# lucianpls/QB3

Measured on AMD Instinct MI355X. Metric: MPixel/s encode+decode (QB3M_FTL, 8-bit 3-band), higher is better.
Workload: dtype u8; 1 GPU; 16384x16384x3 uint8 NOISY3 seed 2; QB3M_FTL qb3x_encode_device (self-indexed container, table level 2) + qb3x_decode_device of that container alone (index = NULL, restart table inside the container); table_level=2, container_bytes=458870207

## Files before the change

### include/qb3x.h

```cpp
#ifndef QB3_AMD_QB3X_H
#define QB3_AMD_QB3X_H
#include "QB3.h"

#if defined(__cplusplus)
extern "C" {
#endif

int qb3x_device_count(void);

void qb3x_trim(void);

unsigned qb3x_last_decode_status(const decsp p);

size_t qb3x_index_size(const encsp p);
size_t qb3x_decoder_index_size(const decsp p);

size_t qb3x_encode_device(encsp p, const void *d_src, void *d_dst, void *d_index, void *stream);

size_t qb3x_decode_device(decsp p, const void *d_src, void *d_dst, const void *d_index, void *stream);

size_t qb3x_decode_window_device(decsp p, const void *d_src, const void *d_index, size_t x0, size_t y0, size_t w, size_t h,
                                 void *d_dst, size_t dst_stride, void *stream);
size_t qb3x_read_window(decsp p, size_t x0, size_t y0, size_t w, size_t h, void *dst, size_t dst_stride);
size_t qb3x_window_segments(const decsp p, size_t x0, size_t y0, size_t w, size_t h, size_t *blocks_per_segment);
int    qb3x_last_window_path(const decsp p);
size_t qb3x_last_window_segments(const decsp p);
#define QB3X_WINK_U16 1u
#define QB3X_WINK_CF8 2u
#define QB3X_WINK_UNIT 4u
#define QB3X_WINK_CFU 8u
void qb3x_set_decoder_window_kernels(decsp p, unsigned mask);

// ... 75 lines not shown
```

### qb3_amd/__init__.py

```python
import ctypes as C
import os

_HERE = os.path.dirname(os.path.abspath(__file__))
LIB_PATH = os.environ.get("QB3_LIB_PATH") or os.path.join(_HERE, "libQB3.so")

if not os.path.exists(LIB_PATH):
    raise ImportError(f"{LIB_PATH} not built: run `python -c 'import __graft_entry__ as g; g.build()'` "
                      "or `make -C qb3_amd/csrc` (there is no CPU fallback)")

try:
    import torch as _torch
except ImportError:
    _torch = None

lib = C.CDLL(LIB_PATH)

QB3_U8, QB3_I8, QB3_U16, QB3_I16, QB3_U32, QB3_I32, QB3_U64, QB3_I64 = range(8)
QB3M_BASE_Z, QB3M_CF, QB3M_RLE, QB3M_CF_RLE, QB3M_BASE_H, QB3M_CF_H, QB3M_RLE_H, QB3M_CF_RLE_H, QB3M_FTL = range(9)
QB3M_DEFAULT, QB3M_BASE, QB3M_BEST, QB3M_STORED, QB3M_INVALID = 8, 4, 7, 255, -1
QB3X_REF_CBAND0 = 1
QB3X_WINK_U16 = 1
QB3X_WINK_CF8 = 2
QB3X_WINK_UNIT = 4
QB3X_WINK_CFU = 8
# ... 35 lines not shown
    "qb3_read_info": (C.c_bool, [_vp]),
    "qb3_read_data": (_sz, [_vp, _vp]),
    "qb3_destroy_decoder": (None, [_vp]),
    "qb3_decoded_size": (_sz, [_vp]),
    "qb3_get_type": (C.c_int, [_vp]),
    "qb3_set_decoder_stride": (None, [_vp, _sz]),
    "qb3_get_mode": (C.c_int, [_vp]),
    "qb3_get_quanta": (_u64, [_vp]),
    "qb3_get_order": (_u64, [_vp]),
    "qb3_get_coreband": (C.c_bool, [_vp, C.POINTER(_sz)]),
    "qb3x_device_count": (C.c_int, []),
    "qb3x_trim": (None, []),
    "qb3x_last_decode_status": (C.c_uint, [_vp]),
    "qb3x_index_size": (_sz, [_vp]),
    "qb3x_set_encoder_index_chunk": (None, [_vp, C.c_int]),
    "qb3x_decoder_index_size": (_sz, [_vp]),
    "qb3x_encode_device": (_sz, [_vp, _vp, _vp, _vp, _vp]),
    "qb3x_decode_device": (_sz, [_vp, _vp, _vp, _vp, _vp]),
    "qb3x_encode_tiles": (_sz, [_vp, _vp, _sz, _sz, _vp, _sz, _vp, C.POINTER(_sz), _vp]),
    "qb3x_decode_tiles": (_sz, [_vp, _vp, _sz, _sz, C.POINTER(_sz), _vp, _sz, _vp, _vp]),
    "qb3x_decode_tile_ok": (C.c_int, [_vp, _sz]),
    "qb3x_mosaic_tiles": (_sz, [_sz, _sz, _sz, _sz, C.POINTER(_sz), C.POINTER(_sz)]),
    "qb3x_encode_mosaic": (_sz, [_vp, _vp, _sz, _sz, _sz, _vp, _sz, _vp, C.POINTER(_sz), _vp]),
    "qb3x_decode_mosaic": (_sz, [_vp, _vp, _sz, C.POINTER(_sz), _sz, _sz, _vp, _sz, _vp, _vp]),
    "qb3x_mosaic_window_tiles": (_sz, [_sz] * 8 + [C.POINTER(_sz)] * 4),
    "qb3x_decode_mosaic_windows": (_sz, [_vp, _vp, _sz, C.POINTER(_sz), _sz, _sz, _vp, _sz, _vp]),
    "qb3x_last_mosaic_whole_tiles": (_sz, [_vp]),
    "qb3x_decode_window_device": (_sz, [_vp, _vp, _vp, _sz, _sz, _sz, _sz, _vp, _sz, _vp]),
    "qb3x_read_window": (_sz, [_vp, _sz, _sz, _sz, _sz, _vp, _sz]),
    "qb3x_window_segments": (_sz, [_vp, _sz, _sz, _sz, _sz, C.POINTER(_sz)]),
# ... 266 lines not shown
```

### qb3_amd/csrc/api_mem.cpp

```cpp
#include <chrono>
#include <mutex>
#include "qb3_host.h"

using namespace qb3dev;
using namespace qb3api;

struct DevPool {
    struct Item { void *p; size_t cap; int dev; };
    static constexpr size_t POOL_ITEMS = 24;
    const size_t POOL_BYTES = [] { const char *e = getenv("QB3_POOL_MB"); return (e && e[0] ? (size_t)strtoull(e, nullptr, 10) : (size_t)3072) << 20; }();
    std::mutex mu;
    std::vector<Item> items;
    size_t bytes = 0;
    void *take(size_t n, int dev, size_t *cap) {
        std::lock_guard<std::mutex> l(mu);
        size_t best = items.size();
        for (size_t i = 0; i < items.size(); i++)
            if (items[i].dev == dev && items[i].cap >= n && items[i].cap / 2 <= n && (best == items.size() || items[i].cap < items[best].cap)) best = i;
        if (best == items.size()) return nullptr;
        void *p = items[best].p;
        *cap = items[best].cap;
        bytes -= items[best].cap;
        items.erase(items.begin() + (long)best);
        return p;
// ... 50 lines not shown
}
QB3_API void qb3x_trim(void) { try { dev_pool().trim(); qb3host::ring_trim(); } catch (...) {} }

bool qb3api::device_ok() {
    int n = 0;
    hipError_t e = hipGetDeviceCount(&n);
    if (e != hipSuccess || n <= 0) { set_error("no usable HIP device (the block codec has no CPU fallback)", (int)e); return false; }
    return true;
}

hipError_t qb3api::wait_stream(hipStream_t st) {
    const auto t0 = std::chrono::steady_clock::now();
    for (uint32_t i = 0;; i++) {
        const hipError_t e = hipStreamQuery(st);
        if (e != hipErrorNotReady) return e;
        if ((i & 63) == 63 && std::chrono::steady_clock::now() - t0 > std::chrono::milliseconds(4)) break;
    }
    return hipStreamSynchronize(st);
}
hipError_t qb3api::fetch_small(void *dst, const void *d_src, size_t n, hipStream_t st) {
    static thread_local void *pinned = nullptr;
    if (!pinned && hipHostMalloc(&pinned, 1024, hipHostMallocDefault) != hipSuccess) pinned = nullptr;
    if (!pinned || n > 1024) {
        hipError_t e = hipMemcpyAsync(dst, d_src, n, hipMemcpyDeviceToHost, st);
        return e == hipSuccess ? hipStreamSynchronize(st) : e;
    }
    hipError_t e = hipMemcpyAsync(pinned, d_src, n, hipMemcpyDeviceToHost, st);
    if (e == hipSuccess) e = wait_stream(st);
    if (e == hipSuccess) memcpy(dst, pinned, n);
    return e;
}

static void parallel_memcpy(uint8_t *dst, const uint8_t *src, size_t n) {
// ... 73 lines not shown
```

### qb3_amd/csrc/api_tiles.cpp

```cpp
#include "qb3_host.h"

using namespace qb3dev;
using namespace qb3api;

static const uint8_t *grid_img(const TileGrid &G, size_t u) { return (const uint8_t *)G.img + (u / G.cols) * G.img_row + (u % G.cols) * G.img_col; }
static size_t grid_k(const TileGrid &G, size_t u) { return G.k0 + (u / G.cols) * G.k_row + u % G.cols; }
static size_t grid_piece(const TileGrid &G, size_t first, size_t batch, uint32_t *cols) {
    const size_t c = first % G.cols;
    if (c == 0 && batch >= G.cols) {
        *cols = (uint32_t)G.cols;
        return std::min(batch / G.cols, (G.n - first) / G.cols) * G.cols;
    }
    *cols = 0;
    return std::min(batch, G.cols - c);
}
template <class H> struct StrideGuard {
    H *p; size_t saved;
    explicit StrideGuard(H *h) : p(h), saved(h->stride) {}
    ~StrideGuard() { p->stride = saved; }
};

static size_t encode_tiles_loop(encsp p, const TileGrid &G, size_t first, size_t n, void *d_dst, size_t dst_pitch,
                                void *d_index, size_t isz, size_t *sizes, void *stream, qb3_mode mode) {
    size_t done = 0;
// ... 2 lines not shown
        qb3_reset_encoder(p);
        p->mode = mode;
        sizes[k] = qb3x_encode_device(p, grid_img(G, u), (uint8_t *)d_dst + k * dst_pitch,
                                      d_index ? (uint8_t *)d_index + k * isz : nullptr, stream);
        done += sizes[k] != 0;
    }
    return done;
}

size_t qb3api::encode_tile_grids(encsp p, const TileGrid *grids, size_t ngrids, void *d_dst, size_t dst_pitch,
                                 void *d_index, size_t *sizes, void *stream) {
    const size_t isz = d_index ? qb3x_index_size(p) : 0;
    const qb3_mode mode = p->mode;
    const size_t tsz = szof(p->type);
    hipStream_t st = (hipStream_t)stream;
    StrideGuard<encs> keep(p);
    size_t nmax = 0;
    for (size_t gi = 0; gi < ngrids; gi++) nmax = std::max(nmax, grids[gi].n);
    const bool batchable = !is_rle_mode(mode) && mode != QB3M_STORED && p->quanta < 2 && p->xsize >= 4 && p->ysize >= 4 &&
                           p->xsize * p->ysize > 16 && !p->error && device_ok();
    if (!batchable) {
        size_t k = 0;
        for (size_t gi = 0; gi < ngrids; gi++) {
            p->stride = grids[gi].stride;
            k += encode_tiles_loop(p, grids[gi], 0, grids[gi].n, d_dst, dst_pitch, d_index, isz, sizes, stream, mode);
        }
        if (mode != QB3M_STORED) p->mode = mode;
        return k;
    }

// ... 205 lines not shown
```

### qb3_amd/csrc/k_enc_post.hip

```cpp
#include "qb3_kernels.h"
#include "qb3_ix_fill.h"

namespace qb3dev {

__global__ void __launch_bounds__(SCAN_GROUP / 4) enc_scan_kernel(const EncArgs a0) {
    const EncArgs a = enc_for_tile(a0, blockIdx.y);
    __shared__ uint32_t wsum[16];
    __shared__ uint64_t wsum64[16];
    __shared__ uint64_t carry;
    __shared__ uint32_t is_last;
    const uint32_t tid = threadIdx.x, i0 = blockIdx.x * SCAN_GROUP + 4 * tid;
    const uint32_t ngroups = (a.nchunks + SCAN_GROUP - 1) / SCAN_GROUP;
    uint32_t v[4], sum = 0;
#pragma unroll
    for (int k = 0; k < 4; k++) { v[k] = (i0 + k < a.nchunks) ? a.chunk_bits[i0 + k] : 0; sum += v[k]; }
    uint32_t total;
    uint64_t off = block_exscan(sum, wsum, &total);
#pragma unroll
    for (int k = 0; k < 4; k++) if (i0 + k < a.nchunks) { a.chunk_off[i0 + k] = off; off += v[k]; }
    if (tid == 0) {
        a.group_sum[blockIdx.x] = total;
        __threadfence();
        is_last = atomicAdd((uint32_t *)&a.group_sum[ngroups + 1], 1u) == gridDim.x - 1;
        carry = 0;
    }
    __syncthreads();
    if (!is_last) return;
    __threadfence();
    for (uint32_t base = 0; base < ngroups; base += blockDim.x) {
        const uint32_t i = base + tid;
        const uint64_t g = i < ngroups ? __hip_atomic_load(&a.group_sum[i], __ATOMIC_RELAXED, __HIP_MEMORY_SCOPE_AGENT) : 0ull;
        const uint64_t ex = block_exscan_v<uint64_t>(g, wsum64);
        const uint64_t c0 = carry;
        if (i < ngroups) a.group_sum[i] = c0 + ex;
        __syncthreads();
        if (tid == blockDim.x - 1) carry = c0 + ex + g;
        __syncthreads();
    }
    if (tid == 0) { a.group_sum[ngroups] = carry; a.res->zero_run = 0; a.res->ff_pairs = 0; a.res->zero_dwords = 0; }
}

__device__ __forceinline__ uint64_t chunk_start(const EncArgs &a, uint32_t k) {
    if (k >= a.nchunks) return a.group_sum[(a.nchunks + SCAN_GROUP - 1) / SCAN_GROUP];
    return a.group_sum[k / SCAN_GROUP] + a.chunk_off[k];
}

__device__ __forceinline__ uint32_t zero_runs_in(uint32_t cur, uint32_t nxt) {
    return (uint32_t)(cur == 0) + (uint32_t)(__builtin_amdgcn_alignbit(nxt, cur, 8) == 0) +
           (uint32_t)(__builtin_amdgcn_alignbit(nxt, cur, 16) == 0) + (uint32_t)(__builtin_amdgcn_alignbit(nxt, cur, 24) == 0);
}
__device__ __forceinline__ uint32_t ff_pairs_in(uint32_t v) {
    const uint32_t t = v & (v >> 8) & 0x00ffffffu;
    return (uint32_t)__popc(((t & 0x7f7f7fu) + 0x010101u) & t & 0x808080u);
}
// ... 326 lines not shown
```

### qb3_amd/csrc/k_host.hip

```cpp
#include "qb3_kernels.h"
#include "qb3_walk.h"

namespace qb3dev {

static thread_local char g_err[256] = "";
const char *last_error() { return g_err; }
void set_error(const char *what, int e) {
    snprintf(g_err, sizeof(g_err), "%s: %s", what, e ? hipGetErrorString((hipError_t)e) : "failed");
}

const Tuning &tuning() {
    static const Tuning t = [] {
        auto on = [](const char *name) { const char *e = getenv(name); return e && e[0] && e[0] != '0'; };
        Tuning v;
        v.no_px = on("QB3_NO_PX");
        v.slow_walk = on("QB3_SLOW_WALK");
        const char *cap = getenv("QB3_WALK_TAB_KB");
        v.walk_tab_kb = cap ? (size_t)strtoull(cap, nullptr, 10) : 0;
        v.slow_index = on("QB3_SLOW_INDEX");
        { const char *e = getenv("QB3_WIDE_BAND"); v.wide_band = e && e[0] ? atoi(e) : 0; }
        v.no_bl = on("QB3_NO_BLOCK_LENGTHS");
        { const char *e = getenv("QB3_BEST_SAMPLE_MIN"); v.best_sample_min = e && e[0] ? (uint32_t)strtoul(e, nullptr, 10) : BEST_SAMPLE_MIN; }
        { const char *e = getenv("QB3_EXITS_FROM"); v.exits_from = e && e[0] ? (int64_t)strtoll(e, nullptr, 10) : -1; }
        return v;
// ... 4 lines not shown
}
#include <map>
#include <mutex>
#include <string>
#include <vector>
namespace qb3dev {
struct ProfPending { const char *name; hipEvent_t a, b; };
static std::mutex g_prof_mu;
static int g_prof_level = 0;
static std::vector<ProfPending> g_prof_pending;
static std::vector<hipEvent_t> g_prof_pool;
static std::map<std::string, std::pair<double, uint64_t>> g_prof_acc;
void prof_enable(int level) { std::lock_guard<std::mutex> l(g_prof_mu); g_prof_level = level; }
static bool prof_minor(const char *n) { const std::string s(n); return s == "enc_scan" || s == "enc_seams" || s == "enc_best_scan" || s == "enc_best_recode"; }
void prof_reset() { std::lock_guard<std::mutex> l(g_prof_mu); g_prof_acc.clear(); }
static hipEvent_t prof_event() {
    if (!g_prof_pool.empty()) { hipEvent_t e = g_prof_pool.back(); g_prof_pool.pop_back(); return e; }
    hipEvent_t e = nullptr;
    (void)hipEventCreate(&e);
    return e;
}
ProfScope::ProfScope(const char *n, hipStream_t s) : st(s), name(n) {
    std::lock_guard<std::mutex> l(g_prof_mu);
    on = g_prof_level == 1 || (g_prof_level == 2 && !prof_minor(n)) || (g_prof_level >= 3 && std::string(n).find("_units") != std::string::npos);
    if (on) { a = prof_event(); b = prof_event(); (void)hipEventRecord(a, st); }
}
ProfScope::~ProfScope() {
    if (!on) return;
    (void)hipEventRecord(b, st);
    std::lock_guard<std::mutex> l(g_prof_mu);
// ... 265 lines not shown
    a.magic_dpr = magic_div(a.dpr); a.magic_bands = magic_div(g.bands);
    uint8_t *w = (uint8_t *)ws;
    const EncWs L = enc_ws_layout(g, plan.nchunks, plan.nbp, plan.threads);
    a.chunk_bits = (uint32_t *)(w + L.bits);
    a.chunk_off = (uint64_t *)(w + L.off);
    a.group_sum = (uint64_t *)(w + L.gsum);
    a.seams = (uint32_t *)(w + L.seams);
    a.scratch = (uint32_t *)(w + L.scratch);
    a.cw_has = w + L.cwhas; a.cw_val = (uint64_t *)(w + L.cwval); a.centry = (uint64_t *)(w + L.centry); a.centry_parts = (uint32_t *)(w + L.cparts); a.recode_n = a.centry_parts + 32 * MAXBANDS;
    a.cw_used = w + L.cwused; a.seg_from_entry = w + L.segfe; a.recode_need = (uint32_t *)(w + L.rneed); a.recode_list = (uint32_t *)(w + L.rlist);
    a.slot_dw = L.slot_dw;
    a.px_ng = plan.px16 ? plan.px16_ng : 1; a.px_magic_ng = magic_div(a.px_ng);
    a.px16_bg = g.tsz == 2 ? px16_bands_per_lane(g) : 0;
    a.px_aligned = !(g.w & 3) && !((g.stride * g.tsz) & 3) && !((uintptr_t)img & 3) && !(tile_pitch_bits(tg, false) & 3);
    a.res = (EncResult *)(w + L.res);
    a.st = st_in;
    a.ix_bl = ix.base && ix.block_lens;
    a.ix_coder = a.ix_bl && plan.px && g.tsz == 1 && g.mode != CM_BEST && g.seg_blocks == 64 && ix.blocks == 64;
    a.ix_wgs = 0;
    a.have_idx = index != nullptr && !(a.ix_coder && ix.own_index);
    a.idx_no_ulen = index && ix.base && ix.own_index && !ix.block_lens;
    a.idx = index ? index_view(g, index) : IndexView{nullptr, nullptr, nullptr, nullptr, nullptr};
    if (g.tsz != 1 && g.tsz != 2 && g.tsz != 4 && g.tsz != 8) { set_error("encode: bad value size", 0); return false; }
    return true;
}

int launch_encode(const Geometry &g, const EncPlan &plan, const void *img, uint32_t *out32, uint32_t out_bit0,
                  const BandState &st_in, void *ws, void *index, void *stream, const TileBatch &tb,
                  const uint8_t *hdr, uint32_t hdr_len, const IxTable &ix, bool zrun_probe) {
    EncArgs a;
    if (!make_enc_args(a, g, plan, img, out32, out_bit0, st_in, ws, index, tb, hdr, hdr_len, ix, zrun_probe)) return -1;
    return launch_encode_all(a, plan, (hipStream_t)stream);
}

bool encode_strips_ok(const Geometry &g, const EncPlan &plan) { return g.mode != CM_BEST && plan.nchunks > 2 * SCAN_GROUP; }
uint32_t encode_strip_count(const EncPlan &plan) { return (plan.nchunks + SCAN_GROUP - 1) / SCAN_GROUP; }
uint64_t encode_strip_blocks(const EncPlan &plan, uint32_t strip) {
    const uint64_t c = std::min<uint64_t>(plan.nchunks, ((uint64_t)strip + 1) * SCAN_GROUP);
    return c * plan.nbp;
}
const uint64_t *encode_strip_total(const Geometry &g, const EncPlan &plan, void *ws, uint32_t strip) {
    const EncWs L = enc_ws_layout(g, plan.nchunks, plan.nbp, plan.threads);
    return (const uint64_t *)((uint8_t *)ws + L.gsum) + strip + 1;
}
int launch_encode_strip(const Geometry &g, const EncPlan &plan, const void *img, uint32_t *out32, uint32_t out_bit0,
                        const BandState &st_in, void *ws, void *index, void *stream, const uint8_t *hdr, uint32_t hdr_len, const IxTable &ix, uint32_t strip) {
// ... 160 lines not shown
```

### qb3_amd/csrc/qb3_api.cpp

```cpp
#include <chrono>
#include <new>
#include <limits>
#include <thread>
#include "qb3_host.h"

using namespace qb3dev;
using namespace qb3api;

static size_t raw_size(const encs *p) { return p->xsize * p->ysize * p->nbands * szof(p->type); }

static CodecMode codec_mode(int mode) {
    if (mode == QB3M_FTL) return CM_FTL;
    if (mode == QB3M_BASE_H || mode == QB3M_BASE_Z || mode == QB3M_RLE || mode == QB3M_RLE_H) return CM_BASE;
    return CM_BEST;
}

Geometry qb3api::make_geometry(size_t w, size_t h, size_t bands, int dtype, size_t stride, uint64_t order, int mode,
                              const size_t *cband_sz, const uint8_t *cband_u8) {
    Geometry g;
    memset(&g, 0, sizeof(g));
    g.w = (uint32_t)w; g.h = (uint32_t)h; g.bands = (uint32_t)bands; g.tsz = (uint32_t)szof(dtype);
    g.stride = stride ? stride : w * bands;
    g.order = order ? order : HILBERT;
    g.nbx = (uint32_t)((w + 3) / 4); g.nby = (uint32_t)((h + 3) / 4);
// ... 16 lines not shown
    { const char *e = getenv("QB3X_INDEX_CHUNK"); p->ix_chunk = e ? (atoi(e) >= 2 ? 2 : atoi(e) != 0) : 0; }
    for (size_t c = 0; c < QB3_MAXBANDS; c++) p->cband[c] = c < b ? c : 0;
    if (b == 3 || b == 4) p->cband[0] = p->cband[2] = 1;
    qb3_reset_encoder(p);
    return p;
}

QB3_API void qb3_reset_encoder(encsp p) {
    for (size_t c = 0; c < QB3_MAXBANDS; c++) p->band[c].prev = p->band[c].runbits = p->band[c].cf = 0;
    p->error = 0;
}

QB3_API void qb3_destroy_encoder(encsp p) {
    if (!p) return;
    release_all({&p->d_img, &p->d_out, &p->d_ws, &p->d_q, &p->d_idx, &p->d_rle, &p->d_mos});
    p->stager.release(); p->stager2.release(); p->pipe.release();
    delete p;
}

QB3_API bool qb3_set_encoder_coreband(encsp p, size_t b, size_t *bands) {
    if (b != p->nbands) return false;
    for (size_t i = 0; i < b; i++) p->cband[i] = (uint8_t)((bands[i] < b) ? bands[i] : i);
    for (size_t i = 0; i < b; i++) if (p->cband[i] != i) p->cband[p->cband[i]] = p->cband[i];
    for (size_t i = 0; i < b; i++) bands[i] = p->cband[i];
    return true;
}

QB3_API void qb3_set_encoder_stride(encsp p, size_t stride) { p->stride = stride; }

QB3_API bool qb3_set_encoder_quanta(encsp p, uint64_t q, bool away) {
// ... 51 lines not shown


static size_t stored_encode_host(encsp p, const void *source, void *destination) {
    uint8_t *d = (uint8_t *)destination;
    p->mode = QB3M_STORED;
    const size_t hdr = write_headers(p, d);
    if (p->error) return 0;
    const size_t tsz = szof(p->type), line = p->xsize * p->nbands * tsz;
    const size_t stride = (p->stride ? p->stride : p->xsize * p->nbands) * tsz;
    for (size_t y = 0; y < p->ysize; y++) memcpy(d + hdr + y * line, (const uint8_t *)source + y * stride, line);
    return hdr + raw_size(p);
}

static bool encode_blocks_device(encsp p, const Geometry &g, const void *d_img, uint8_t *d_out, size_t hdr,
                                 void *d_index, hipStream_t st, bool carry, uint64_t *bits, const uint8_t *hdrbytes,
                                 size_t hdr_stamp, const IxTable &ix, int *zero_run = nullptr) {
    EncPlan plan = plan_encode(g, ((uintptr_t)d_img & (g.tsz - 1)) == 0);
    if (!p->d_ws.ensure(plan.ws_bytes)) return false;
    BandState bs;
    memset(&bs, 0, sizeof(bs));
    for (size_t c = 0; c < p->nbands; c++) {
        bs.prev[c] = p->band[c].prev; bs.cf[c] = p->band[c].cf; bs.rung[c] = (uint8_t)p->band[c].runbits;
    }
    uint32_t *out32 = (uint32_t *)(d_out + (hdr & ~(size_t)3));
    EncResult res;
    const uint8_t *dres = (const uint8_t *)p->d_ws.p + plan.ws_bytes - sizeof(EncResult);
    if (launch_encode(g, plan, d_img, out32, (uint32_t)(8 * (hdr & 3)), bs, p->d_ws.p, d_index, st, TileBatch(), hdrbytes, (uint32_t)hdr_stamp, ix, zero_run != nullptr)) return false;
    const hipError_t e = fetch_small(&res, dres, sizeof(res), st);
    if (e != hipSuccess) { set_error("encode kernels", (int)e); return false; }
    prof_collect();
    *bits = res.total_bits;
    { static const bool dbg = getenv("QB3_DEBUG_RLE") != nullptr; if (dbg && zero_run) fprintf(stderr, "encode: zero_run %llu ff_pairs %llu zero_dwords %llu (%u chunks)\n", (unsigned long long)res.zero_run, (unsigned long long)res.ff_pairs, (unsigned long long)res.zero_dwords, plan.nchunks); }
    if (zero_run) *zero_run = rle0_may_win(res) ? (rle0_no_uniform_chunk(res, (uint64_t)plan.nbp * g.bands / 4) ? 2 : 1) : 0;
    if (carry)
        for (size_t c = 0; c < p->nbands; c++) {
            p->band[c].prev = (size_t)res.prev[c]; p->band[c].runbits = res.rung[c]; p->band[c].cf = (size_t)res.cf[c];
        }
    return true;
}

struct ModeGuard {
    encs *p; qb3_mode mode; bool armed = true;
    ModeGuard(encs *h) : p(h), mode(h->mode) {}
    ~ModeGuard() { if (armed) p->mode = mode; }
// ... 106 lines not shown
    prof_collect();
    *bits_out = res_host->total_bits;
    if (carry)
        for (size_t c = 0; c < p->nbands; c++) {
            p->band[c].prev = (size_t)res_host->prev[c]; p->band[c].runbits = res_host->rung[c]; p->band[c].cf = (size_t)res_host->cf[c];
        }
    return 1;
}

static size_t encode_common(encsp p, const void *host_src, void *host_dst, const void *d_src, void *d_dst,
                            void *d_index, hipStream_t st) {
    const bool on_host = host_src != nullptr;
    const size_t tsz = szof(p->type), line = p->xsize * p->nbands * tsz;
    const size_t src_stride_bytes = (p->stride ? p->stride : p->xsize * p->nbands) * tsz;
    const size_t src_span = src_stride_bytes * (p->ysize - 1) + line;
    if (p->xsize * p->ysize <= 16) {
        if (on_host) return stored_encode_host(p, host_src, host_dst);
        std::vector<uint8_t> tmp(src_span), out(64 + raw_size(p));
        if (!device_ok()) { p->error = QB3E_LIBERR; return 0; }
        HIPOK(hipMemcpyAsync(tmp.data(), d_src, tmp.size(), hipMemcpyDeviceToHost, st));
        HIPOK(hipStreamSynchronize(st));
        size_t n = stored_encode_host(p, tmp.data(), out.data());
        HIPOK(hipMemcpyAsync(d_dst, out.data(), n, hipMemcpyHostToDevice, st));
        HIPOK(hipStreamSynchronize(st));
        return n;
    }
    ModeGuard guard(p);
    const qb3_mode mode = p->mode;
    const bool rle = is_rle_mode(mode);
    const size_t ixroom = mode == QB3M_STORED ? 0 : ix_room(p);
// ... 51 lines not shown
    size_t hdr_stamp = hdr;
    if (ixroom && !narrow) {
        ixt = ix_layout(g, p->ix_chunk);
        hdr_stamp = write_headers(p, hdrbuf, false);
        hdr = hdr_stamp + ix_total_bytes(ixt) + 2;
        ixt.base = out_dev + hdr_stamp;
        if (!d_index) {
            if (!p->d_idx.ensure(index_bytes(g))) { p->error = QB3E_LIBERR; return 0; }
            d_index = p->d_idx.p;
            ixt.own_index = true;
        }
    }
    uint64_t bits = 0;
    int has_run = 1;
    bool piped = false;
    if (want_pipe) {
        const int r = encode_pipelined(p, g, host_src, host_dst, src_span, line, out_dev, hdr, hdrbuf, hdr_stamp, ixt, d_index, carry, &bits);
        if (r < 0) return 0;
        piped = r > 0;
        if (!piped && !upload_now()) { p->error = QB3E_LIBERR; return 0; }
    }
    if (!piped && !encode_blocks_device(p, g, img_dev, out_dev, hdr, d_index, st, carry, &bits, hdrbuf, hdr_stamp, ixt, rle ? &has_run : nullptr)) {
        p->error = QB3E_LIBERR; return 0;
    }
    p->error = 0;
    const size_t len = hdr + (size_t)((bits + 7) / 8);
    const size_t len_ref = len - (ixt.base ? ix_total_bytes(ixt) : 0);

    if (rle) {
        p->mode = mode;
        if (len_ref <= maxsz / 2 && has_run) {
            const size_t n = len - hdr;
            uint64_t rsz64 = 0;
            if (!p->d_rle.ensure(rle0_ws_bytes(n)) || rle0_device_size(out_dev + hdr, n, p->d_rle.p, false, &rsz64, st, has_run == 2)) { p->error = QB3E_LIBERR; return 0; }
            const size_t rsz = (size_t)rsz64;
            if (rsz <= maxsz - len_ref && rsz < n) {
                uint8_t hdr2[80];
// ... 7 lines not shown
                } else {
                    if (tbl && h2 != hdr_stamp) HIPOK(hipMemcpyAsync((uint8_t *)d_dst + h2, out_dev + hdr_stamp, tbl, hipMemcpyDeviceToDevice, st));
                    HIPOK(hipMemcpyAsync((uint8_t *)d_dst + h2 + tbl, p->d_q.p, rsz, hipMemcpyDeviceToDevice, st));
                    HIPOK(hipMemcpyAsync(d_dst, hdr2, h2, hipMemcpyHostToDevice, st));
                    HIPOK(hipStreamSynchronize(st));
                }
                return h2 + tbl + rsz;
            }
        }
    }
    if (raw_size(p) > len_ref) {
        if (on_host) {
            memcpy(host_dst, hdrbuf, hdr_stamp);
            if (!piped && !download(p->stager, (uint8_t *)host_dst + hdr_stamp, out_dev + hdr_stamp, len - hdr_stamp, st)) { p->error = QB3E_LIBERR; return 0; }
        }
        return len;
    }
    guard.armed = false;
    if (on_host) return stored_encode_host(p, host_src, host_dst);
    p->mode = QB3M_STORED;
    const size_t h2 = write_headers(p, hdrbuf);
    HIPOK(hipMemcpyAsync(d_dst, hdrbuf, h2, hipMemcpyHostToDevice, st));
    HIPOK(hipMemcpy2DAsync((uint8_t *)d_dst + h2, line, d_src, src_stride_bytes, line, p->ysize, hipMemcpyDeviceToDevice, st));
    HIPOK(hipStreamSynchronize(st));
    return h2 + raw_size(p);
}

QB3_API size_t qb3_encode(encsp p, void *source, void *destination) {
    if (!p || !source || !destination) return 0;
    return abi_guard<size_t>(0, [&] { return encode_common(p, source, destination, nullptr, nullptr, nullptr, nullptr); });
}

QB3_API size_t qb3x_encode_device(encsp p, const void *d_src, void *d_dst, void *d_index, void *stream) {
    if (!p || !d_src || !d_dst || ((uintptr_t)d_dst & 3)) { if (p) p->error = QB3E_EINV; return 0; }
    return abi_guard<size_t>(0, [&] { return encode_common(p, nullptr, nullptr, d_src, d_dst, d_index, (hipStream_t)stream); });
}

QB3_API void qb3x_set_encoder_index_chunk(encsp p, int on) { if (p) p->ix_chunk = on >= 2 ? 2 : on != 0; }

QB3_API size_t qb3x_index_size(const encsp p) {
    if (!p || p->xsize < 4 || p->ysize < 4) return 0;
    Geometry g = make_geometry(p->xsize, p->ysize, p->nbands, p->type, p->stride, p->order, p->mode, p->cband, nullptr);
    return index_bytes(g);
}

QB3_API void qb3_destroy_decoder(decsp p) {
    if (!p) return;
    release_all({&p->d_in, &p->d_img, &p->d_ws, &p->d_ix, &p->d_rle, &p->d_tab, &p->d_win, &p->d_wst, &p->d_wout, &p->d_wsrc, &p->d_wdesc, &p->d_rg, &p->d_wfull, &p->d_wgat, &p->d_mos});
    p->h_wdesc.release(); p->h_wst.release(); p->h_rg.release(); p->h_wgat.release();
    p->stager.release(); p->stager2.release(); p->pipe.release();
    delete p;
// ... 308 lines not shown
    DevBuf ws;
    if (!ws.ensure(rle0_ws_bytes(n))) return 0;
    uint64_t total = 0;
    size_t ret = 0;
    if (rle0_device_size(d_src, n, ws.p, decode != 0, &total, stream) == 0) {
        if (!d_dst) ret = (size_t)total;
        else if (total <= dst_cap && rle0_device_write(d_src, n, ws.p, decode != 0, d_dst, stream) == 0 &&
                 hipStreamSynchronize((hipStream_t)stream) == hipSuccess) ret = (size_t)total;
    }
    ws.release();
    return ret;
}
QB3_API void qb3x_profile_enable(int level) { prof_enable(level < 0 ? 0 : level); }
QB3_API void qb3x_profile_reset(void) { prof_reset(); }
QB3_API int qb3x_profile_get(const char *kernel, double *total_ms, uint64_t *count) { return prof_get(kernel, total_ms, count) ? 1 : 0; }
QB3_API int qb3x_profile_names(char *buf, size_t bufsize) { return prof_names(buf, bufsize); }

QB3_API decsp qb3_create_decoder(void *source, size_t source_size, size_t *image_size) {
    decsp p = qb3_read_start(source, source_size, image_size);
    if (p && !qb3_read_info(p)) { qb3_destroy_decoder(p); p = nullptr; }
    return p;
}
QB3_API size_t qb3_decode(decsp p, void *destination) { return qb3_read_data(p, destination); }
```

### qb3_amd/csrc/qb3_dev.h

```cpp
#pragma once
#include <stddef.h>
#include <stdint.h>
#include <algorithm>
#include <vector>

namespace qb3dev {

constexpr int MAXBANDS = 16;
constexpr uint64_t ZCURVE = 0x0145236789cdabefull;
constexpr uint64_t HILBERT = 0x01548cd9aefb7623ull;

enum CodecMode { CM_FTL = 0, CM_BASE = 1, CM_BEST = 2 };

struct Geometry {
    uint32_t w, h, bands, tsz;
    uint64_t stride;
    uint64_t order;
    uint32_t nbx, nby;
    uint64_t nblocks;
    uint32_t mode;
    uint32_t seg_blocks;
    uint64_t nseg;
    uint32_t ulen_sz;
    uint8_t cband[MAXBANDS];
// ... 33 lines not shown

constexpr uint64_t WIN_LAUNCH_WAVES = 1ull << 24;
inline bool window_unit_geometry_ok(const Geometry &g) {
    return g.seg_blocks && (uint64_t)g.nby * (g.nbx / g.seg_blocks + 2) <= WIN_LAUNCH_WAVES && g.nblocks < (1ull << 31);
}

struct EncResult {
    uint64_t total_bits;
    uint64_t prev[MAXBANDS];
    uint64_t cf[MAXBANDS];
    uint32_t rung[MAXBANDS];
    uint64_t zero_run;
    uint64_t ff_pairs;
    uint64_t zero_dwords;
};

inline bool rle0_may_win(const EncResult &r) { return r.zero_run > 0 && 2 * r.zero_run + 2 > r.ff_pairs; }
inline bool rle0_no_uniform_chunk(const EncResult &r, uint64_t min_chunk_bytes) {
    if (min_chunk_bytes < 16) return false;
    const uint64_t shared = 2 * (4096 / min_chunk_bytes + 2);
    return shared < 1000 && r.zero_dwords < 1022 - shared && r.ff_pairs < 1024;
}

struct EncPlan {
    uint32_t threads;
    uint32_t slots;
    uint32_t nchunks;
    size_t lds_bytes;
    size_t ws_bytes;
    uint32_t nbp;
// ... 41 lines not shown
    uint32_t cols = 0; uint64_t src_row = 0, dst_row = 0, idx_row = 0; };
struct TileGridRule { uint32_t cols, magic; uint64_t src, src_row, dst, dst_row, idx, idx_row; };
TileGridRule make_tile_grid(const TileBatch &tb);
inline uint64_t tile_pitch_bits(const TileGridRule &r, bool dst) { return dst ? (r.dst | r.dst_row) : (r.src | r.src_row); }
size_t walk_table_bytes(uint32_t ntiles, uint64_t max_bits, uint32_t tsz);
size_t walk_table_min_bytes(uint32_t ntiles, uint32_t tsz);
size_t walk_memory_bytes(const Geometry &g, uint32_t ntiles, uint64_t max_bits);
size_t walk_table_cap();
struct DecPlan;
bool walk_table_applies(const Geometry &g, const DecPlan &plan);

int launch_encode(const Geometry &g, const EncPlan &plan, const void *img, uint32_t *out32, uint32_t out_bit0,
                  const BandState &st_in, void *ws, void *index, void *stream, const TileBatch &tb = TileBatch(),
                  const uint8_t *hdr = nullptr, uint32_t hdr_len = 0,
                  const IxTable &ix = IxTable(),
                  bool zrun_probe = false);

bool encode_strips_ok(const Geometry &g, const EncPlan &plan);
uint32_t encode_strip_count(const EncPlan &plan);
uint64_t encode_strip_blocks(const EncPlan &plan, uint32_t strip);
const uint64_t *encode_strip_total(const Geometry &g, const EncPlan &plan, void *ws, uint32_t strip);
int launch_encode_strip(const Geometry &g, const EncPlan &plan, const void *img, uint32_t *out32, uint32_t out_bit0,
                        const BandState &st_in, void *ws, void *index, void *stream, const uint8_t *hdr, uint32_t hdr_len, const IxTable &ix, uint32_t strip);
int launch_encode_tail(const Geometry &g, const EncPlan &plan, const void *img, uint32_t *out32, uint32_t out_bit0,
                       const BandState &st_in, void *ws, void *index, void *stream, const uint8_t *hdr, uint32_t hdr_len, const IxTable &ix);

struct DecPlan {
    uint32_t threads;
    uint32_t nwg;
    size_t lds_bytes;
    size_t ws_bytes;
// ... 98 lines not shown

int launch_reindex_fill(const Geometry &g, void *index, const IxTable &ix, void *stream);
int launch_reindex_finish(const Geometry &g, const IxTable &ix, const uint8_t *hdr, size_t hdr_len, void *d_dst, const void *d_src, void *d_pay, uint64_t n, void *stream);
constexpr size_t DEC_WS_INDEX_OFF = 64;

size_t rle0_ws_bytes(uint64_t n);
int rle0_device_size(const void *d_src, uint64_t n, void *ws, bool decode, uint64_t *total, void *stream, bool no_uniform_chunk = false);
int rle0_device_write(const void *d_src, uint64_t n, void *ws, bool decode, void *d_dst, void *stream);


int launch_quantize(void *dst, const void *src, const Geometry &g, int dtype, uint64_t q, bool away, void *stream);
int launch_dequantize(void *img, const Geometry &g, int dtype, uint64_t q, void *stream);

void prof_enable(int level);
void prof_reset();
void prof_collect();
bool prof_get(const char *name, double *total_ms, uint64_t *count);
int  prof_names(char *buf, size_t bufsize);

const char *last_error();
void set_error(const char *what, int hip_err);

}
```

### qb3_amd/csrc/qb3_host.h

```cpp
#pragma once
#include <hip/hip_runtime_api.h>
#include <cstring>
#include <cstdlib>
#include <cstdio>
#include <exception>
#include <initializer_list>
#include <vector>
#include <utility>
#include <algorithm>
#include "../../include/QB3.h"
#include "../../include/qb3x.h"
#include "qb3_dev.h"
#include "qb3_host_io.h"

#define QB3_API extern "C" __attribute__((visibility("default")))
#define HIPOK(x) do { hipError_t e_ = (x); if (e_ != hipSuccess) { qb3dev::set_error(#x, (int)e_); p->error = QB3E_LIBERR; return 0; } } while (0)

struct DevBuf {
    void *p = nullptr;
    size_t cap = 0;
    int dev = 0;
    bool ensure(size_t n);
    void release(bool idle = false);
};
struct PinBuf {
    void *p = nullptr;
    size_t cap = 0;
    bool ensure(size_t n) {
// ... 37 lines not shown

struct encs {
    size_t xsize, ysize, nbands, stride;
    uint64_t order, quanta;
    band_state band[QB3_MAXBANDS];
    size_t cband[QB3_MAXBANDS];
    int error;
    qb3_mode mode;
    qb3_dtype type;
    bool away;
    int ix_chunk;
    DevBuf d_img, d_out, d_ws, d_q, d_idx, d_rle;
    DevBuf d_mos;
    Stager stager, stager2;
    Pipe pipe;
};

struct decs {
    size_t xsize, ysize, nbands, stride;
    uint64_t order, quanta;
    int error, stage;
    uint8_t cband[QB3_MAXBANDS];
    qb3_mode mode;
    qb3_dtype type;
    uint8_t *s_in;
    size_t s_size;
    uint8_t *s_start;
    bool saw_cb;
    unsigned compat;
    size_t hdr_avail;
// ... 39 lines not shown
    constexpr int typesizes[8] = { 1, 1, 2, 2, 4, 4, 8, 8 };
    return (dt < 0 || dt > QB3_I64) ? 0 : typesizes[dt];
}
inline bool is_rle_mode(int m) { return m == QB3M_RLE || m == QB3M_CF_RLE || m == QB3M_RLE_H || m == QB3M_CF_RLE_H; }

template <class R, class F> R abi_guard(R fail, F &&f) noexcept {
    try { return f(); }
    catch (const std::exception &e) { qb3dev::set_error(e.what(), -1); }
    catch (...) { qb3dev::set_error("C++ exception inside the library", -1); }
    return fail;
}

void release_all(std::initializer_list<DevBuf *> bufs);
bool device_ok();
hipError_t wait_stream(hipStream_t st);
hipError_t fetch_small(void *dst, const void *d_src, size_t n, hipStream_t st);
bool upload(Stager &sg, void *d_dst, const void *h_src, size_t bytes, hipStream_t st);
bool download(Stager &sg, void *h_dst, const void *d_src, size_t bytes, hipStream_t st);

size_t write_headers(const encs *p, uint8_t *dst, bool with_dt = true);
decsp read_start_impl(void *source, size_t hdr_avail, size_t source_size, size_t *image_size);
qb3dev::IxTable handle_table(const decs *p, const uint8_t *base);
qb3dev::Geometry decoder_geometry(const decs *p, size_t w, size_t h, size_t stride);

struct TileGrid {
    size_t n, cols;
    const void *img;
    size_t img_col, img_row;
    size_t stride;
    size_t k0, k_row;
// ... 43 lines not shown
```

### qb3_amd/csrc/qb3_kernels.h

```cpp
#pragma once
#include <hip/hip_runtime.h>
#include <algorithm>
#include <type_traits>
#include "qb3_dev.h"

namespace qb3dev {

template <typename T> struct UBits { static constexpr uint32_t v = sizeof(T) == 1 ? 3 : sizeof(T) == 2 ? 4 : sizeof(T) == 4 ? 5 : 6; };

template <typename T> __device__ __forceinline__ T mags_t(T v) {
    constexpr uint32_t B = 8 * sizeof(T);
    return (T)((T)(v << 1) ^ (T)(0 - (T)(v >> (B - 1))));
}
template <typename T> __device__ __forceinline__ T smag_t(T v) {
    return (T)((T)(v >> 1) ^ (T)(0 - (T)(v & 1)));
}
template <typename T> __device__ __forceinline__ T mabs_t(T v) { return (T)((v >> 1) + (v & 1)); }
template <typename T> __device__ __forceinline__ T mmul_t(T v, T m) { return (T)((T)(mabs_t<T>(v) * (T)(m << 1)) - (T)(v & 1)); }
__device__ __forceinline__ uint32_t topbit64(uint64_t v) { return 63u - (uint32_t)__clzll((long long)v); }
__device__ __forceinline__ uint32_t topbit32(uint32_t v) { return 31u - (uint32_t)__clz((int)v); }
template <typename T> __device__ __forceinline__ uint32_t topbit_t(T v) {
    if (sizeof(T) == 8) return topbit64((uint64_t)v | 1);
    return topbit32((uint32_t)v | 1);
}
// ... 141 lines not shown
    uint32_t tcols, tmagic;
    uint64_t tr_img, tr_out, tr_idx;
    uint32_t hdr_len;
    uint32_t hdr_back;
    uint8_t hdr[80];
    uint32_t px_ng, px_magic_ng;
    uint32_t px16_bg;
    uint32_t px_aligned;
    uint8_t *ix_dst;
    uint32_t ix_K, ix_spe, ix_E;
    uint32_t ix_bl;
    uint32_t ix_per_chunk, ix_blocks;
    uint32_t ix_coder;
    uint32_t ix_wgs;
    EncResult *res;
    BandState st;
    IndexView idx;
    uint32_t have_idx;
    uint32_t zrun_probe;
    uint32_t idx_no_ulen;
    uint32_t chunk0, chunk_end;
    uint32_t finish_what;
};


template <typename P> __device__ __forceinline__ P *shift_ptr(P *p, uint64_t bytes) { return p ? (P *)((uint8_t *)p + bytes) : p; }
__device__ __forceinline__ EncArgs enc_for_tile(EncArgs a, uint32_t t) {
    if (t) {
        const uint32_t r = __umulhi(t, a.tmagic), c = t - r * a.tcols;
        a.img = (const uint8_t *)a.img + (r * a.tr_img + c * a.ts_img);
// ... 386 lines not shown
```

### qb3_amd/device.py

```python
import ctypes as C

import numpy as np
import torch

from . import lib, last_error, TYPESIZE, NP_DTYPE, QB3M_FTL, _sz, window_array, band_array, RangedReader

_vp = C.c_void_p


def _stream_ptr():
    return _vp(torch.cuda.current_stream().cuda_stream)


class DeviceEncoder:

    def __init__(self, w, h, bands, dtype, mode=QB3M_FTL, cband=None, want_index=True, index_chunk=False):
        self.w, self.h, self.bands, self.dtype = w, h, bands, dtype
        self.p = lib.qb3_create_encoder(w, h, bands, dtype)
        if not self.p:
            raise ValueError("qb3_create_encoder refused the parameters")
        self.mode = lib.qb3_set_encoder_mode(self.p, mode)
        if index_chunk:
            lib.qb3x_set_encoder_index_chunk(self.p, int(index_chunk))
        if cband is not None:
            arr = (_sz * bands)(*cband)
            lib.qb3_set_encoder_coreband(self.p, bands, arr)
        self.max_size = lib.qb3_max_encoded_size(self.p)
        self.raw_bytes = w * h * bands * TYPESIZE[dtype]
        self.index_bytes = lib.qb3x_index_size(self.p) if want_index else 0
        self.dst = None
        self.index = None

    def close(self):
        if self.p and lib is not None:
            lib.qb3_destroy_encoder(self.p)
            self.p = None

    __del__ = close

    def encode(self, src, dst=None, index=None):
        assert src.is_cuda and src.is_contiguous() and src.numel() * src.element_size() >= self.raw_bytes
        if dst is None:
            if self.dst is None:
                self.dst = torch.empty((self.max_size + 3) // 4 * 4, dtype=torch.uint8, device=src.device)
            dst = self.dst
        if index is None and self.index_bytes:
            if self.index is None:
                self.index = torch.empty(self.index_bytes, dtype=torch.uint8, device=src.device)
            index = self.index
        lib.qb3_reset_encoder(self.p)
        lib.qb3_set_encoder_mode(self.p, self.mode)
        n = lib.qb3x_encode_device(self.p, _vp(src.data_ptr()), _vp(dst.data_ptr()),
                                   _vp(index.data_ptr()) if index is not None else None, _stream_ptr())
# ... 317 lines not shown
```

Measured before the change: 312,900 MPixel/s.

## Publish encode length via mapped host record and return before stream drains

The scan kernel now writes the final bit length, band state and a sequence number into a pinned, host-mapped record with a system-scope release store. The host spins on that word and can return from encode as soon as the length is known, leaving later tail kernels queued on the stream instead of doing a full device-to-host fetch and stream sync. Async tail is enabled by default from the Python DeviceEncoder, and later calls on other streams settle any pending tail first. This aims to cut host-side synchronisation latency per encode. The risk is that host-visible memory polling and same-stream ordering have to keep the decode correct.

New measurement: 315,400 MPixel/s (median of 6 runs). No clear change (+0.8%).

```diff
diff --git a/include/qb3x.h b/include/qb3x.h
--- a/include/qb3x.h
+++ b/include/qb3x.h
@@ -16,6 +16,9 @@
 size_t qb3x_decoder_index_size(const decsp p);
 
 size_t qb3x_encode_device(encsp p, const void *d_src, void *d_dst, void *d_index, void *stream);
+
+void qb3x_set_encoder_async_tail(encsp p, int on);
+int  qb3x_encoder_tail_pending(const encsp p);
 
 size_t qb3x_decode_device(decsp p, const void *d_src, void *d_dst, const void *d_index, void *stream);
 
diff --git a/qb3_amd/__init__.py b/qb3_amd/__init__.py
--- a/qb3_amd/__init__.py
+++ b/qb3_amd/__init__.py
@@ -73,6 +73,8 @@
     "qb3x_last_decode_status": (C.c_uint, [_vp]),
     "qb3x_index_size": (_sz, [_vp]),
     "qb3x_set_encoder_index_chunk": (None, [_vp, C.c_int]),
+    "qb3x_set_encoder_async_tail": (None, [_vp, C.c_int]),
+    "qb3x_encoder_tail_pending": (C.c_int, [_vp]),
     "qb3x_decoder_index_size": (_sz, [_vp]),
     "qb3x_encode_device": (_sz, [_vp, _vp, _vp, _vp, _vp]),
     "qb3x_decode_device": (_sz, [_vp, _vp, _vp, _vp, _vp]),
diff --git a/qb3_amd/csrc/api_mem.cpp b/qb3_amd/csrc/api_mem.cpp
--- a/qb3_amd/csrc/api_mem.cpp
+++ b/qb3_amd/csrc/api_mem.cpp
@@ -88,9 +88,32 @@
     for (uint32_t i = 0;; i++) {
         const hipError_t e = hipStreamQuery(st);
         if (e != hipErrorNotReady) return e;
-        if ((i & 63) == 63 && std::chrono::steady_clock::now() - t0 > std::chrono::milliseconds(4)) break;
+        if ((i & 63) == 63 && std::chrono::steady_clock::now() - t0 > WAIT_POLL) break;
     }
     return hipStreamSynchronize(st);
+}
+
+bool qb3api::enc_record_ready(encs *p) {
+    if (p->rec) return true;
+    if (p->rec_failed) return false;
+    void *h = nullptr, *d = nullptr;
+    if (hipHostMalloc(&h, sizeof(EncRecord), hipHostMallocMapped | hipHostMallocCoherent) != hipSuccess || hipHostGetDevicePointer(&d, h, 0) != hipSuccess) {
+        (void)hipGetLastError();
+        if (h) (void)hipHostFree(h);
+        p->rec_failed = true;
+        return false;
+    }
+    memset(h, 0, sizeof(EncRecord));
+    p->rec = (EncRecord *)h; p->rec_dev = (EncRecord *)d;
+    return true;
+}
+void qb3api::enc_record_release(encs *p) {
+    if (p->rec) (void)hipHostFree(p->rec);
+    p->rec = p->rec_dev = nullptr;
+}
+void qb3api::enc_settle_tail(encs *p, hipStream_t st) {
+    if (p->tail_queued && p->tail_stream != st) { (void)hipStreamSynchronize(p->tail_stream); p->tail_queued = false; }
+    p->tail_pending = false;
 }
 hipError_t qb3api::fetch_small(void *dst, const void *d_src, size_t n, hipStream_t st) {
     static thread_local void *pinned = nullptr;
diff --git a/qb3_amd/csrc/api_tiles.cpp b/qb3_amd/csrc/api_tiles.cpp
--- a/qb3_amd/csrc/api_tiles.cpp
+++ b/qb3_amd/csrc/api_tiles.cpp
@@ -40,6 +40,7 @@
     const qb3_mode mode = p->mode;
     const size_t tsz = szof(p->type);
     hipStream_t st = (hipStream_t)stream;
+    enc_settle_tail(p, st);
     StrideGuard<encs> keep(p);
     size_t nmax = 0;
     for (size_t gi = 0; gi < ngrids; gi++) nmax = std::max(nmax, grids[gi].n);
diff --git a/qb3_amd/csrc/k_enc_post.hip b/qb3_amd/csrc/k_enc_post.hip
--- a/qb3_amd/csrc/k_enc_post.hip
+++ b/qb3_amd/csrc/k_enc_post.hip
@@ -37,7 +37,13 @@
         if (tid == blockDim.x - 1) carry = c0 + ex + g;
         __syncthreads();
     }
-    if (tid == 0) { a.group_sum[ngroups] = carry; a.res->zero_run = 0; a.res->ff_pairs = 0; a.res->zero_dwords = 0; }
+    if (tid == 0) {
+        a.group_sum[ngroups] = carry; a.res->zero_run = 0; a.res->ff_pairs = 0; a.res->zero_dwords = 0;
+        if (a.rec) {
+            for (uint32_t c = 0; c < a.g.bands; c++) { a.rec->prev[c] = a.res->prev[c]; a.rec->cf[c] = a.res->cf[c]; a.rec->rung[c] = a.res->rung[c]; }
+            __hip_atomic_store(&a.rec->word, ((uint64_t)a.rec_seq << ENC_REC_LEN_BITS) | carry, __ATOMIC_RELEASE, __HIP_MEMORY_SCOPE_SYSTEM);
+        }
+    }
 }
 
 __device__ __forceinline__ uint64_t chunk_start(const EncArgs &a, uint32_t k) {
diff --git a/qb3_amd/csrc/k_host.hip b/qb3_amd/csrc/k_host.hip
--- a/qb3_amd/csrc/k_host.hip
+++ b/qb3_amd/csrc/k_host.hip
@@ -42,6 +42,7 @@
 void prof_enable(int level) { std::lock_guard<std::mutex> l(g_prof_mu); g_prof_level = level; }
 static bool prof_minor(const char *n) { const std::string s(n); return s == "enc_scan" || s == "enc_seams" || s == "enc_best_scan" || s == "enc_best_recode"; }
 void prof_reset() { std::lock_guard<std::mutex> l(g_prof_mu); g_prof_acc.clear(); }
+bool prof_times_tail() { std::lock_guard<std::mutex> l(g_prof_mu); return g_prof_level == 1 || g_prof_level == 2; }
 static hipEvent_t prof_event() {
     if (!g_prof_pool.empty()) { hipEvent_t e = g_prof_pool.back(); g_prof_pool.pop_back(); return e; }
     hipEvent_t e = nullptr;
@@ -337,6 +338,7 @@
     a.px16_bg = g.tsz == 2 ? px16_bands_per_lane(g) : 0;
     a.px_aligned = !(g.w & 3) && !((g.stride * g.tsz) & 3) && !((uintptr_t)img & 3) && !(tile_pitch_bits(tg, false) & 3);
     a.res = (EncResult *)(w + L.res);
+    a.rec = nullptr; a.rec_seq = 0;
     a.st = st_in;
     a.ix_bl = ix.base && ix.block_lens;
     a.ix_coder = a.ix_bl && plan.px && g.tsz == 1 && g.mode != CM_BEST && g.seg_blocks == 64 && ix.blocks == 64;
@@ -350,9 +352,10 @@
 
 int launch_encode(const Geometry &g, const EncPlan &plan, const void *img, uint32_t *out32, uint32_t out_bit0,
                   const BandState &st_in, void *ws, void *index, void *stream, const TileBatch &tb,
-                  const uint8_t *hdr, uint32_t hdr_len, const IxTable &ix, bool zrun_probe) {
+                  const uint8_t *hdr, uint32_t hdr_len, const IxTable &ix, bool zrun_probe, EncRecord *rec, uint32_t rec_seq) {
     EncArgs a;
     if (!make_enc_args(a, g, plan, img, out32, out_bit0, st_in, ws, index, tb, hdr, hdr_len, ix, zrun_probe)) return -1;
+    if (!tb.n) { a.rec = rec; a.rec_seq = rec_seq; }
     return launch_encode_all(a, plan, (hipStream_t)stream);
 }
 
diff --git a/qb3_amd/csrc/qb3_api.cpp b/qb3_amd/csrc/qb3_api.cpp
--- a/qb3_amd/csrc/qb3_api.cpp
+++ b/qb3_amd/csrc/qb3_api.cpp
@@ -54,6 +54,7 @@
 QB3_API void qb3_destroy_encoder(encsp p) {
     if (!p) return;
     release_all({&p->d_img, &p->d_out, &p->d_ws, &p->d_q, &p->d_idx, &p->d_rle, &p->d_mos});
+    enc_record_release(p);
     p->stager.release(); p->stager2.release(); p->pipe.release();
     delete p;
 }
@@ -135,7 +136,7 @@
 
 static bool encode_blocks_device(encsp p, const Geometry &g, const void *d_img, uint8_t *d_out, size_t hdr,
                                  void *d_index, hipStream_t st, bool carry, uint64_t *bits, const uint8_t *hdrbytes,
-                                 size_t hdr_stamp, const IxTable &ix, int *zero_run = nullptr) {
+                                 size_t hdr_stamp, const IxTable &ix, int *zero_run = nullptr, bool *early = nullptr) {
     EncPlan plan = plan_encode(g, ((uintptr_t)d_img & (g.tsz - 1)) == 0);
     if (!p->d_ws.ensure(plan.ws_bytes)) return false;
     BandState bs;
@@ -146,9 +147,25 @@
     uint32_t *out32 = (uint32_t *)(d_out + (hdr & ~(size_t)3));
     EncResult res;
     const uint8_t *dres = (const uint8_t *)p->d_ws.p + plan.ws_bytes - sizeof(EncResult);
-    if (launch_encode(g, plan, d_img, out32, (uint32_t)(8 * (hdr & 3)), bs, p->d_ws.p, d_index, st, TileBatch(), hdrbytes, (uint32_t)hdr_stamp, ix, zero_run != nullptr)) return false;
-    const hipError_t e = fetch_small(&res, dres, sizeof(res), st);
-    if (e != hipSuccess) { set_error("encode kernels", (int)e); return false; }
+    const bool by_record = !zero_run && enc_record_ready(p);
+    if (by_record) p->rec_seq = p->rec_seq % 0xffffu + 1;
+    if (launch_encode(g, plan, d_img, out32, (uint32_t)(8 * (hdr & 3)), bs, p->d_ws.p, d_index, st, TileBatch(), hdrbytes, (uint32_t)hdr_stamp, ix, zero_run != nullptr,
+                      by_record ? p->rec_dev : nullptr, p->rec_seq)) return false;
+    hipError_t e;
+    if (by_record) {
+        memset(&res, 0, sizeof(res));
+        e = wait_record(&p->rec->word, p->rec_seq, ENC_REC_LEN_BITS, st, &res.total_bits);
+        (void)hipGetLastError();
+        if (e == hipSuccess)
+            for (size_t c = 0; c < p->nbands; c++) { res.prev[c] = p->rec->prev[c]; res.cf[c] = p->rec->cf[c]; res.rung[c] = p->rec->rung[c]; }
+        if (e == hipSuccess && early) { *early = true; p->tail_queued = true; p->tail_stream = st; }
+        else if (e == hipSuccess) {
+            e = wait_stream(st);
+            if (e != hipSuccess) set_error("encode kernels", (int)e);
+            if (p->tail_stream == st) p->tail_queued = false;
+        }
+    } else if ((e = fetch_small(&res, dres, sizeof(res), st)) != hipSuccess) set_error("encode kernels", (int)e);
+    if (e != hipSuccess) return false;
     prof_collect();
     *bits = res.total_bits;
     { static const bool dbg = getenv("QB3_DEBUG_RLE") != nullptr; if (dbg && zero_run) fprintf(stderr, "encode: zero_run %llu ff_pairs %llu zero_dwords %llu (%u chunks)\n", (unsigned long long)res.zero_run, (unsigned long long)res.ff_pairs, (unsigned long long)res.zero_dwords, plan.nchunks); }
@@ -285,6 +302,7 @@
     const size_t tsz = szof(p->type), line = p->xsize * p->nbands * tsz;
     const size_t src_stride_bytes = (p->stride ? p->stride : p->xsize * p->nbands) * tsz;
     const size_t src_span = src_stride_bytes * (p->ysize - 1) + line;
+    enc_settle_tail(p, st);
     if (p->xsize * p->ysize <= 16) {
         if (on_host) return stored_encode_host(p, host_src, host_dst);
         std::vector<uint8_t> tmp(src_span), out(64 + raw_size(p));
@@ -366,13 +384,15 @@
     uint64_t bits = 0;
     int has_run = 1;
     bool piped = false;
+    const bool may_return_early = p->async_tail && !on_host && !rle && p->quanta < 2 && !narrow && !prof_times_tail();
+    bool early = false;
     if (want_pipe) {
         const int r = encode_pipelined(p, g, host_src, host_dst, src_span, line, out_dev, hdr, hdrbuf, hdr_stamp, ixt, d_index, carry, &bits);
         if (r < 0) return 0;
         piped = r > 0;
         if (!piped && !upload_now()) { p->error = QB3E_LIBERR; return 0; }
     }
-    if (!piped && !encode_blocks_device(p, g, img_dev, out_dev, hdr, d_index, st, carry, &bits, hdrbuf, hdr_stamp, ixt, rle ? &has_run : nullptr)) {
+    if (!piped && !encode_blocks_device(p, g, img_dev, out_dev, hdr, d_index, st, carry, &bits, hdrbuf, hdr_stamp, ixt, rle ? &has_run : nullptr, may_return_early ? &early : nullptr)) {
         p->error = QB3E_LIBERR; return 0;
     }
     p->error = 0;
@@ -410,6 +430,7 @@
             memcpy(host_dst, hdrbuf, hdr_stamp);
             if (!piped && !download(p->stager, (uint8_t *)host_dst + hdr_stamp, out_dev + hdr_stamp, len - hdr_stamp, st)) { p->error = QB3E_LIBERR; return 0; }
         }
+        p->tail_pending = early;
         return len;
     }
     guard.armed = false;
@@ -419,6 +440,7 @@
     HIPOK(hipMemcpyAsync(d_dst, hdrbuf, h2, hipMemcpyHostToDevice, st));
     HIPOK(hipMemcpy2DAsync((uint8_t *)d_dst + h2, line, d_src, src_stride_bytes, line, p->ysize, hipMemcpyDeviceToDevice, st));
     HIPOK(hipStreamSynchronize(st));
+    if (p->tail_stream == st) p->tail_queued = false;
     return h2 + raw_size(p);
 }
 
@@ -431,6 +453,9 @@
     if (!p || !d_src || !d_dst || ((uintptr_t)d_dst & 3)) { if (p) p->error = QB3E_EINV; return 0; }
     return abi_guard<size_t>(0, [&] { return encode_common(p, nullptr, nullptr, d_src, d_dst, d_index, (hipStream_t)stream); });
 }
+
+QB3_API void qb3x_set_encoder_async_tail(encsp p, int on) { if (p) p->async_tail = on != 0; }
+QB3_API int qb3x_encoder_tail_pending(const encsp p) { return p && p->tail_pending ? 1 : 0; }
 
 QB3_API void qb3x_set_encoder_index_chunk(encsp p, int on) { if (p) p->ix_chunk = on >= 2 ? 2 : on != 0; }
 
@@ -769,7 +794,7 @@
 QB3_API void qb3x_profile_enable(int level) { prof_enable(level < 0 ? 0 : level); }
 QB3_API void qb3x_profile_reset(void) { prof_reset(); }
 QB3_API int qb3x_profile_get(const char *kernel, double *total_ms, uint64_t *count) { return prof_get(kernel, total_ms, count) ? 1 : 0; }
-QB3_API int qb3x_profile_names(char *buf, size_t bufsize) { return prof_names(buf, bufsize); }
+QB3_API int qb3x_profile_names(char *buf, size_t bufsize) { prof_collect(); return prof_names(buf, bufsize); }
 
 QB3_API decsp qb3_create_decoder(void *source, size_t source_size, size_t *image_size) {
     decsp p = qb3_read_start(source, source_size, image_size);
diff --git a/qb3_amd/csrc/qb3_dev.h b/qb3_amd/csrc/qb3_dev.h
--- a/qb3_amd/csrc/qb3_dev.h
+++ b/qb3_amd/csrc/qb3_dev.h
@@ -71,6 +71,14 @@
     uint64_t ff_pairs;
     uint64_t zero_dwords;
 };
+
+struct EncRecord {
+    uint64_t prev[MAXBANDS];
+    uint64_t cf[MAXBANDS];
+    uint32_t rung[MAXBANDS];
+    uint64_t word;
+};
+constexpr uint32_t ENC_REC_LEN_BITS = 48;
 
 inline bool rle0_may_win(const EncResult &r) { return r.zero_run > 0 && 2 * r.zero_run + 2 > r.ff_pairs; }
 inline bool rle0_no_uniform_chunk(const EncResult &r, uint64_t min_chunk_bytes) {
@@ -142,7 +150,8 @@
                   const BandState &st_in, void *ws, void *index, void *stream, const TileBatch &tb = TileBatch(),
                   const uint8_t *hdr = nullptr, uint32_t hdr_len = 0,
                   const IxTable &ix = IxTable(),
-                  bool zrun_probe = false);
+                  bool zrun_probe = false,
+                  EncRecord *rec = nullptr, uint32_t rec_seq = 0);
 
 bool encode_strips_ok(const Geometry &g, const EncPlan &plan);
 uint32_t encode_strip_count(const EncPlan &plan);
@@ -271,6 +280,7 @@
 
 void prof_enable(int level);
 void prof_reset();
+bool prof_times_tail();
 void prof_collect();
 bool prof_get(const char *name, double *total_ms, uint64_t *count);
 int  prof_names(char *buf, size_t bufsize);
diff --git a/qb3_amd/csrc/qb3_host.h b/qb3_amd/csrc/qb3_host.h
--- a/qb3_amd/csrc/qb3_host.h
+++ b/qb3_amd/csrc/qb3_host.h
@@ -12,6 +12,7 @@
 #include "../../include/qb3x.h"
 #include "qb3_dev.h"
 #include "qb3_host_io.h"
+#include "qb3_wait.h"
 
 #define QB3_API extern "C" __attribute__((visibility("default")))
 #define HIPOK(x) do { hipError_t e_ = (x); if (e_ != hipSuccess) { qb3dev::set_error(#x, (int)e_); p->error = QB3E_LIBERR; return 0; } } while (0)
@@ -79,6 +80,13 @@
     DevBuf d_mos;
     Stager stager, stager2;
     Pipe pipe;
+    qb3dev::EncRecord *rec = nullptr, *rec_dev = nullptr;
+    bool rec_failed = false;
+    uint32_t rec_seq = 0;
+    bool async_tail = false;
+    bool tail_pending = false;
+    bool tail_queued = false;
+    hipStream_t tail_stream = nullptr;
 };
 
 struct decs {
@@ -148,6 +156,9 @@
 void release_all(std::initializer_list<DevBuf *> bufs);
 bool device_ok();
 hipError_t wait_stream(hipStream_t st);
+bool enc_record_ready(encs *p);
+void enc_record_release(encs *p);
+void enc_settle_tail(encs *p, hipStream_t st);
 hipError_t fetch_small(void *dst, const void *d_src, size_t n, hipStream_t st);
 bool upload(Stager &sg, void *d_dst, const void *h_src, size_t bytes, hipStream_t st);
 bool download(Stager &sg, void *h_dst, const void *d_src, size_t bytes, hipStream_t st);
diff --git a/qb3_amd/csrc/qb3_kernels.h b/qb3_amd/csrc/qb3_kernels.h
--- a/qb3_amd/csrc/qb3_kernels.h
+++ b/qb3_amd/csrc/qb3_kernels.h
@@ -179,6 +179,8 @@
     uint32_t ix_coder;
     uint32_t ix_wgs;
     EncResult *res;
+    EncRecord *rec;
+    uint32_t rec_seq;
     BandState st;
     IndexView idx;
     uint32_t have_idx;
diff --git a/qb3_amd/csrc/qb3_wait.h b/qb3_amd/csrc/qb3_wait.h
--- /dev/null
+++ b/qb3_amd/csrc/qb3_wait.h
@@ -0,0 +1,40 @@
+#pragma once
+#include <hip/hip_runtime_api.h>
+#include <chrono>
+#include <cstdint>
+
+namespace qb3dev { void set_error(const char *what, int hip_err); }
+
+namespace qb3api {
+
+constexpr std::chrono::milliseconds WAIT_POLL(4);
+
+inline void cpu_relax() {
+#if defined(__x86_64__) || defined(__i386__)
+    __builtin_ia32_pause();
+#endif
+}
+
+inline hipError_t wait_record(const uint64_t *word, uint32_t seq, uint32_t len_bits, hipStream_t st, uint64_t *payload) {
+    auto published = [&] {
+        const uint64_t v = __atomic_load_n(word, __ATOMIC_ACQUIRE);
+        if ((uint32_t)(v >> len_bits) != seq) return false;
+        *payload = v & (((uint64_t)1 << len_bits) - 1);
+        return true;
+    };
+    auto never = [] { qb3dev::set_error("encode: the stream finished without publishing the stream length", 0); return hipErrorUnknown; };
+    const auto t0 = std::chrono::steady_clock::now();
+    for (uint32_t i = 1;; i++) {
+        if (published()) return hipSuccess;
+        if (i & 31) { cpu_relax(); continue; }
+        const hipError_t e = hipStreamQuery(st);
+        if (e == hipSuccess) return published() ? hipSuccess : never();
+        if (e != hipErrorNotReady) { qb3dev::set_error("encode kernels", (int)e); return e; }
+        if (std::chrono::steady_clock::now() - t0 > WAIT_POLL) break;
+    }
+    const hipError_t e = hipStreamSynchronize(st);
+    if (e != hipSuccess) { qb3dev::set_error("encode kernels", (int)e); return e; }
+    return published() ? hipSuccess : never();
+}
+
+}
diff --git a/qb3_amd/device.py b/qb3_amd/device.py
--- a/qb3_amd/device.py
+++ b/qb3_amd/device.py
@@ -14,7 +14,7 @@
 
 class DeviceEncoder:
 
-    def __init__(self, w, h, bands, dtype, mode=QB3M_FTL, cband=None, want_index=True, index_chunk=False):
+    def __init__(self, w, h, bands, dtype, mode=QB3M_FTL, cband=None, want_index=True, index_chunk=False, async_tail=True):
         self.w, self.h, self.bands, self.dtype = w, h, bands, dtype
         self.p = lib.qb3_create_encoder(w, h, bands, dtype)
         if not self.p:
@@ -25,6 +25,7 @@
         if cband is not None:
             arr = (_sz * bands)(*cband)
             lib.qb3_set_encoder_coreband(self.p, bands, arr)
+        lib.qb3x_set_encoder_async_tail(self.p, int(bool(async_tail)))
         self.max_size = lib.qb3_max_encoded_size(self.p)
         self.raw_bytes = w * h * bands * TYPESIZE[dtype]
         self.index_bytes = lib.qb3x_index_size(self.p) if want_index else 0
@@ -37,6 +38,13 @@
             self.p = None
 
     __del__ = close
+
+    def set_async_tail(self, on):
+        lib.qb3x_set_encoder_async_tail(self.p, int(bool(on)))
+
+    @property
+    def tail_pending(self):
+        return bool(lib.qb3x_encoder_tail_pending(self.p))
 
     def encode(self, src, dst=None, index=None):
         assert src.is_cuda and src.is_contiguous() and src.numel() * src.element_size() >= self.raw_bytes
```
